# westlake-repl/Adapter4Rec

Hardware: NVIDIA B200
Metric: train user-sequences/s (SASRec + BERT-base LoRA r=8 adapter-tuning step: fwd+bwd+allreduce+Adam) (higher is better)
Workload: dtype bf16

## Files before the change

adapter4rec_b200/csrc/attention_small.cu:

```cuda
#include "a4r_common.cuh"
#include "mma_sync.cuh"

namespace {

constexpr int LP = 32;
constexpr int WARPS_PER_CTA = 4;

struct AttnParams {
  const __nv_bfloat16* qkv;
  __nv_bfloat16* out;
  const __nv_bfloat16* dout;
  const void* mask;
  int64_t ld_qkv, ld_out, mask_ld;
  int N, L, heads;
  int mask_dtype;
  const int32_t* cu_seqlens;
  int causal;
  float scale, mask_neg;
  uint32_t drop_thr16;
  float drop_scale;
  uint64_t drop_seed, drop_offset;
};

A4R_DEVICE void prob_dropout(float (&s)[2][4][4], const AttnParams& p, int n, int h, int lane) {
  const int g = lane >> 2, t = lane & 3;
  const uint64_t base = p.drop_offset + (static_cast<uint64_t>(n) * p.heads + h) * (32 * 8);
  const uint64_t seed = rng_seed(p.drop_seed);
#pragma unroll
  for (int mt = 0; mt < 2; ++mt)
#pragma unroll
    for (int hh = 0; hh < 2; ++hh) {
      const int i = mt * 16 + hh * 8 + g;
#pragma unroll
      for (int np = 0; np < 2; ++np) {
        const uint64_t r = rng64(seed, base + static_cast<uint64_t>(i) * 8 + np * 4 + t);
#pragma unroll
        for (int q = 0; q < 2; ++q)
#pragma unroll
          for (int e = 0; e < 2; ++e) {
            float& x = s[mt][np * 2 + q][hh * 2 + e];
            x = rng_keep(r, q * 2 + e, p.drop_thr16) ? x * p.drop_scale : 0.0f;
          }
      }
    }
}

template <int COLS>
struct Tile {
  static constexpr int kChunks = COLS / 8;
  static constexpr int kBytes = LP * COLS * 2;
  A4R_DEVICE static uint32_t off(int row, int chunk) {
    const int x = COLS == 64 ? row : (row >> 1);
    return static_cast<uint32_t>(row * COLS * 2 + (((chunk ^ x) & (kChunks - 1)) << 4));
  }
};

template <int COLS>
A4R_DEVICE void load_a(uint32_t (&a)[4], uint32_t base, int m0, int k0, int lane) {
  const int mi = lane >> 3, r = lane & 7;
  const int row = m0 + r + ((mi & 1) << 3);
  const int chunk = (k0 >> 3) + (mi >> 1);
  ldsm_x4(a, base + Tile<COLS>::off(row, chunk));
}
template <int COLS>
A4R_DEVICE void load_a_t(uint32_t (&a)[4], uint32_t base, int m0, int k0, int lane) {
  const int mi = lane >> 3, r = lane & 7;
  const int row = k0 + r + ((mi >> 1) << 3);
  const int chunk = (m0 >> 3) + (mi & 1);
  ldsm_x4_t(a, base + Tile<COLS>::off(row, chunk));
}
template <int COLS>
A4R_DEVICE void load_b_nk(uint32_t (&b)[4], uint32_t base, int n0, int k0, int lane) {
  const int mi = lane >> 3, r = lane & 7;
  const int row = n0 + r + ((mi >> 1) << 3);
  const int chunk = (k0 >> 3) + (mi & 1);
  ldsm_x4(b, base + Tile<COLS>::off(row, chunk));
}
template <int COLS>
A4R_DEVICE void load_b_kn(uint32_t (&b)[4], uint32_t base, int n0, int k0, int lane) {
  const int mi = lane >> 3, r = lane & 7;
  const int row = k0 + r + ((mi & 1) << 3);
  const int chunk = (n0 >> 3) + (mi >> 1);
  ldsm_x4_t(b, base + Tile<COLS>::off(row, chunk));
}

template <int DH>
A4R_DEVICE void load_tile(uint8_t* tile, const __nv_bfloat16* g, int64_t ld, int L, int lane) {
  constexpr int CH = DH / 8;
  const uint32_t base = smem_u32(tile);
#pragma unroll
  for (int i = lane; i < LP * CH; i += 32) {
    const int row = i / CH, ch = i % CH;
    const bool ok = row < L;
    const __nv_bfloat16* src = g + (ok ? static_cast<int64_t>(row) * ld + ch * 8 : 0);
    const int sz = ok ? 16 : 0;
    asm volatile("cp.async.cg.shared.global [%0], [%1], 16, %2;" ::"r"(base + Tile<DH>::off(row, ch)), "l"(src), "r"(sz)
                 : "memory");
  }
}
A4R_DEVICE void cp_async_wait_all() { asm volatile("cp.async.wait_all;" ::: "memory"); }
template <int DH>
A4R_DEVICE void store_tile(const uint8_t* tile, __nv_bfloat16* g, int64_t ld, int L, int lane) {
  constexpr int CH = DH / 8;
#pragma unroll
  for (int i = lane; i < LP * CH; i += 32) {
    const int row = i / CH, ch = i % CH;
    if (row < L) st_na_v4(g + static_cast<int64_t>(row) * ld + ch * 8, *reinterpret_cast<const uint4*>(tile + Tile<DH>::off(row, ch)));
  }
}
template <int COLS, int NT>
A4R_DEVICE void acc_to_tile(uint8_t* tile, const float (&acc)[2][NT][4], float s0a, float s0b, float s1a, float s1b, int lane) {
  const int g = lane >> 2, t = lane & 3;
#pragma unroll
  for (int mt = 0; mt < 2; ++mt) {
    const float sa = mt == 0 ? s0a : s1a, sb = mt == 0 ? s0b : s1b;
#pragma unroll
    for (int nt = 0; nt < NT; ++nt) {
      const int r0 = mt * 16 + g, col = nt * 8 + 2 * t;
      *reinterpret_cast<uint32_t*>(tile + Tile<COLS>::off(r0, col >> 3) + (col & 7) * 2) =
          pack_bf16x2(acc[mt][nt][0] * sa, acc[mt][nt][1] * sa);
      *reinterpret_cast<uint32_t*>(tile + Tile<COLS>::off(r0 + 8, col >> 3) + (col & 7) * 2) =
          pack_bf16x2(acc[mt][nt][2] * sb, acc[mt][nt][3] * sb);
    }
  }
}

struct SeqSpan {
  int64_t row0, mask0;
  int L;
};
A4R_DEVICE SeqSpan seq_span(const AttnParams& p, int n) {
  SeqSpan s;
  if (p.cu_seqlens != nullptr) {
    const int a = __ldg(p.cu_seqlens + n), b = __ldg(p.cu_seqlens + n + 1);
    s.row0 = a, s.mask0 = a, s.L = b - a;
  } else {
    s.row0 = static_cast<int64_t>(n) * p.L, s.mask0 = static_cast<int64_t>(n) * p.mask_ld, s.L = p.L;
  }
  return s;
}
A4R_DEVICE bool key_valid(const AttnParams& p, const SeqSpan& sq, int j) {
  if (p.mask_dtype == 1) return reinterpret_cast<const int64_t*>(p.mask)[sq.mask0 + j] != 0;
  if (p.mask_dtype == 2) return reinterpret_cast<const float*>(p.mask)[sq.mask0 + j] != 0.0f;
  return true;
}

template <int DH>
A4R_DEVICE void scores_softmax(float (&s)[2][4][4], uint32_t sQ, uint32_t sK, const AttnParams& p, int L, int lane,
                               uint32_t keymask_bits) {
#pragma unroll
  for (int mt = 0; mt < 2; ++mt)
#pragma unroll
    for (int nt = 0; nt < 4; ++nt)
#pragma unroll
      for (int e = 0; e < 4; ++e) s[mt][nt][e] = 0.0f;
#pragma unroll
  for (int k0 = 0; k0 < DH; k0 += 16) {
    uint32_t a0[4], a1[4];
    load_a<DH>(a0, sQ, 0, k0, lane);
    load_a<DH>(a1, sQ, 16, k0, lane);
#pragma unroll
    for (int np = 0; np < 2; ++np) {
      uint32_t b[4];
      load_b_nk<DH>(b, sK, np * 16, k0, lane);
      const uint32_t b0[2] = {b[0], b[1]}, b1[2] = {b[2], b[3]};
      mma_bf16_16816(s[0][np * 2], a0, b0);
      mma_bf16_16816(s[0][np * 2 + 1], a0, b1);
      mma_bf16_16816(s[1][np * 2], a1, b0);
      mma_bf16_16816(s[1][np * 2 + 1], a1, b1);
    }
  }
  const int g = lane >> 2, t = lane & 3;
  float colneg[4][2];
#pragma unroll
  for (int nt = 0; nt < 4; ++nt)
#pragma unroll
    for (int e = 0; e < 2; ++e) {
      const int j = nt * 8 + 2 * t + e;
      colneg[nt][e] = j >= L ? -INFINITY : (((keymask_bits >> j) & 1u) ? 0.0f : p.mask_neg);
    }
#pragma unroll
  for (int mt = 0; mt < 2; ++mt) {
#pragma unroll
    for (int h = 0; h < 2; ++h) {
      const int i = mt * 16 + h * 8 + g;
      float mx = -INFINITY;
#pragma unroll
      for (int nt = 0; nt < 4; ++nt)
#pragma unroll
        for (int e = 0; e < 2; ++e) {
          float v = fmaf(s[mt][nt][h * 2 + e], p.scale, colneg[nt][e]);
          if (p.causal && nt * 8 + 2 * t + e > i && colneg[nt][e] == 0.0f) v += p.mask_neg;
          s[mt][nt][h * 2 + e] = v;
          mx = fmaxf(mx, v);
        }
      mx = fmaxf(mx, __shfl_xor_sync(0xffffffffu, mx, 1));
      mx = fmaxf(mx, __shfl_xor_sync(0xffffffffu, mx, 2));
      float sum = 0.0f;
#pragma unroll
      for (int nt = 0; nt < 4; ++nt)
#pragma unroll
        for (int e = 0; e < 2; ++e) {
          const float ex = __expf(s[mt][nt][h * 2 + e] - mx);
          s[mt][nt][h * 2 + e] = ex;
          sum += ex;
        }
      sum += __shfl_xor_sync(0xffffffffu, sum, 1);
      sum += __shfl_xor_sync(0xffffffffu, sum, 2);
      const float inv = 1.0f / sum;
#pragma unroll
      for (int nt = 0; nt < 4; ++nt)
#pragma unroll
        for (int e = 0; e < 2; ++e) s[mt][nt][h * 2 + e] *= inv;
    }
  }
}

A4R_DEVICE uint32_t build_keymask(const AttnParams& p, const SeqSpan& sq, int lane) {
  const bool ok = lane < sq.L ? key_valid(p, sq, lane) : false;
  return __ballot_sync(0xffffffffu, ok);
}

A4R_DEVICE void acc_to_a(uint32_t (&a)[4], const float (&c0)[4], const float (&c1)[4]) {
  a[0] = pack_bf16x2(c0[0], c0[1]);
  a[1] = pack_bf16x2(c0[2], c0[3]);
  a[2] = pack_bf16x2(c1[0], c1[1]);
  a[3] = pack_bf16x2(c1[2], c1[3]);
}

template <int DH>
__global__ void __launch_bounds__(WARPS_PER_CTA * 32, 3) attn_fwd_kernel(const AttnParams p) {
  extern __shared__ __align__(128) uint8_t smem_attn[];
  constexpr int TB = Tile<DH>::kBytes;
  const int warp = threadIdx.x >> 5, lane = threadIdx.x & 31;
  uint8_t* my = smem_attn + warp * 3 * TB;
  const int64_t total = static_cast<int64_t>(p.N) * p.heads;
  for (int64_t w = static_cast<int64_t>(blockIdx.x) * WARPS_PER_CTA + warp; w < total;
       w += static_cast<int64_t>(gridDim.x) * WARPS_PER_CTA) {
    const int n = static_cast<int>(w / p.heads), h = static_cast<int>(w % p.heads);
    const int64_t Hd = static_cast<int64_t>(p.heads) * DH;
    const SeqSpan sq = seq_span(p, n);
    const __nv_bfloat16* q = p.qkv + sq.row0 * p.ld_qkv + h * DH;
    load_tile<DH>(my, q, p.ld_qkv, sq.L, lane);
    load_tile<DH>(my + TB, q + Hd, p.ld_qkv, sq.L, lane);
    load_tile<DH>(my + 2 * TB, q + 2 * Hd, p.ld_qkv, sq.L, lane);
    const uint32_t km = build_keymask(p, sq, lane);
    cp_async_wait_all();
    __syncwarp();
    const uint32_t sQ = smem_u32(my), sK = sQ + TB, sV = sK + TB;
    float s[2][4][4];
    scores_softmax<DH>(s, sQ, sK, p, sq.L, lane, km);
    if (p.drop_thr16 != 0) prob_dropout(s, p, n, h, lane);
    float o[2][DH / 8][4];
#pragma unroll
    for (int mt = 0; mt < 2; ++mt)
#pragma unroll
      for (int nt = 0; nt < DH / 8; ++nt)
#pragma unroll
        for (int e = 0; e < 4; ++e) o[mt][nt][e] = 0.0f;
#pragma unroll
    for (int ks = 0; ks < 2; ++ks) {
      uint32_t a0[4], a1[4];
      acc_to_a(a0, s[0][2 * ks], s[0][2 * ks + 1]);
      acc_to_a(a1, s[1][2 * ks], s[1][2 * ks + 1]);
#pragma unroll
      for (int np = 0; np < DH / 16; ++np) {
        uint32_t b[4];
        load_b_kn<DH>(b, sV, np * 16, ks * 16, lane);
        const uint32_t b0[2] = {b[0], b[1]}, b1[2] = {b[2], b[3]};
        mma_bf16_16816(o[0][np * 2], a0, b0);
        mma_bf16_16816(o[0][np * 2 + 1], a0, b1);
        mma_bf16_16816(o[1][np * 2], a1, b0);
        mma_bf16_16816(o[1][np * 2 + 1], a1, b1);
      }
    }
    __syncwarp();
    acc_to_tile<DH, DH / 8>(my, o, 1.f, 1.f, 1.f, 1.f, lane);
    __syncwarp();
    store_tile<DH>(my, p.out + sq.row0 * p.ld_out + h * DH, p.ld_out, sq.L, lane);
    __syncwarp();
  }
}

template <int DH>
__global__ void __launch_bounds__(WARPS_PER_CTA * 32) attn_bwd_kernel(const AttnParams p) {
  extern __shared__ __align__(128) uint8_t smem_attn[];
  constexpr int TB = Tile<DH>::kBytes;
  constexpr int PB = Tile<32>::kBytes;
  const int warp = threadIdx.x >> 5, lane = threadIdx.x & 31;
  uint8_t* my = smem_attn + warp * (4 * TB + 2 * PB);
  const int64_t total = static_cast<int64_t>(p.N) * p.heads;
  for (int64_t w = static_cast<int64_t>(blockIdx.x) * WARPS_PER_CTA + warp; w < total;
       w += static_cast<int64_t>(gridDim.x) * WARPS_PER_CTA) {
    const int n = static_cast<int>(w / p.heads), h = static_cast<int>(w % p.heads);
    const int64_t Hd = static_cast<int64_t>(p.heads) * DH;
    const SeqSpan sq = seq_span(p, n);
    const __nv_bfloat16* q = p.qkv + sq.row0 * p.ld_qkv + h * DH;
    uint8_t *tQ = my, *tK = my + TB, *tV = my + 2 * TB, *tdO = my + 3 * TB, *tP = my + 4 * TB, *tdS = tP + PB;
    load_tile<DH>(tQ, q, p.ld_qkv, sq.L, lane);
    load_tile<DH>(tK, q + Hd, p.ld_qkv, sq.L, lane);
    load_tile<DH>(tV, q + 2 * Hd, p.ld_qkv, sq.L, lane);
    load_tile<DH>(tdO, p.dout + sq.row0 * p.ld_out + h * DH, p.ld_out, sq.L, lane);
    const uint32_t km = build_keymask(p, sq, lane);
    cp_async_wait_all();
    __syncwarp();
    const uint32_t sQ = smem_u32(tQ), sK = smem_u32(tK), sV = smem_u32(tV), sdO = smem_u32(tdO), sP = smem_u32(tP),
                   sdS = smem_u32(tdS);
    float s[2][4][4];
    scores_softmax<DH>(s, sQ, sK, p, sq.L, lane, km);
    float dp[2][4][4];
#pragma unroll
    for (int mt = 0; mt < 2; ++mt)
#pragma unroll
      for (int nt = 0; nt < 4; ++nt)
#pragma unroll
        for (int e = 0; e < 4; ++e) dp[mt][nt][e] = 0.0f;
#pragma unroll
    for (int k0 = 0; k0 < DH; k0 += 16) {
      uint32_t a0[4], a1[4];
      load_a<DH>(a0, sdO, 0, k0, lane);
      load_a<DH>(a1, sdO, 16, k0, lane);
#pragma unroll
      for (int np = 0; np < 2; ++np) {
        uint32_t b[4];
        load_b_nk<DH>(b, sV, np * 16, k0, lane);
        const uint32_t b0[2] = {b[0], b[1]}, b1[2] = {b[2], b[3]};
        mma_bf16_16816(dp[0][np * 2], a0, b0);
        mma_bf16_16816(dp[0][np * 2 + 1], a0, b1);
        mma_bf16_16816(dp[1][np * 2], a1, b0);
        mma_bf16_16816(dp[1][np * 2 + 1], a1, b1);
      }
    }
    float sd[2][4][4];
#pragma unroll
    for (int mt = 0; mt < 2; ++mt)
#pragma unroll
      for (int nt = 0; nt < 4; ++nt)
#pragma unroll
        for (int e = 0; e < 4; ++e) sd[mt][nt][e] = s[mt][nt][e];
    if (p.drop_thr16 != 0) {
      prob_dropout(sd, p, n, h, lane);
#pragma unroll
      for (int mt = 0; mt < 2; ++mt)
#pragma unroll
        for (int nt = 0; nt < 4; ++nt)
#pragma unroll
          for (int e = 0; e < 4; ++e) dp[mt][nt][e] = (sd[mt][nt][e] != 0.0f) ? dp[mt][nt][e] * p.drop_scale : 0.0f;
    }
#pragma unroll
    for (int mt = 0; mt < 2; ++mt)
#pragma unroll
      for (int hh = 0; hh < 2; ++hh) {
        float d = 0.0f;
#pragma unroll
        for (int nt = 0; nt < 4; ++nt)
#pragma unroll
          for (int e = 0; e < 2; ++e) d += s[mt][nt][hh * 2 + e] * dp[mt][nt][hh * 2 + e];
        d += __shfl_xor_sync(0xffffffffu, d, 1);
        d += __shfl_xor_sync(0xffffffffu, d, 2);
#pragma unroll
        for (int nt = 0; nt < 4; ++nt)
#pragma unroll
          for (int e = 0; e < 2; ++e)
            dp[mt][nt][hh * 2 + e] = s[mt][nt][hh * 2 + e] * (dp[mt][nt][hh * 2 + e] - d) * p.scale;
      }
    acc_to_tile<32, 4>(tP, sd, 1.f, 1.f, 1.f, 1.f, lane);
    acc_to_tile<32, 4>(tdS, dp, 1.f, 1.f, 1.f, 1.f, lane);
    __syncwarp();
    float acc[2][DH / 8][4];
#pragma unroll
    for (int mt = 0; mt < 2; ++mt)
#pragma unroll
      for (int nt = 0; nt < DH / 8; ++nt)
#pragma unroll
        for (int e = 0; e < 4; ++e) acc[mt][nt][e] = 0.0f;
#pragma unroll
    for (int ks = 0; ks < 2; ++ks) {
      uint32_t a0[4], a1[4];
      acc_to_a(a0, dp[0][2 * ks], dp[0][2 * ks + 1]);
      acc_to_a(a1, dp[1][2 * ks], dp[1][2 * ks + 1]);
#pragma unroll
      for (int np = 0; np < DH / 16; ++np) {
        uint32_t b[4];
        load_b_kn<DH>(b, sK, np * 16, ks * 16, lane);
        const uint32_t b0[2] = {b[0], b[1]}, b1[2] = {b[2], b[3]};
        mma_bf16_16816(acc[0][np * 2], a0, b0);
        mma_bf16_16816(acc[0][np * 2 + 1], a0, b1);
        mma_bf16_16816(acc[1][np * 2], a1, b0);
        mma_bf16_16816(acc[1][np * 2 + 1], a1, b1);
      }
    }
    float dk[2][DH / 8][4], dv[2][DH / 8][4];
#pragma unroll
    for (int mt = 0; mt < 2; ++mt)
#pragma unroll
      for (int nt = 0; nt < DH / 8; ++nt)
#pragma unroll
        for (int e = 0; e < 4; ++e) dk[mt][nt][e] = dv[mt][nt][e] = 0.0f;
#pragma unroll
    for (int ks = 0; ks < 2; ++ks) {
      uint32_t a0[4], a1[4], p0[4], p1[4];
      load_a_t<32>(a0, sdS, 0, ks * 16, lane);
      load_a_t<32>(a1, sdS, 16, ks * 16, lane);
      load_a_t<32>(p0, sP, 0, ks * 16, lane);
      load_a_t<32>(p1, sP, 16, ks * 16, lane);
#pragma unroll
      for (int np = 0; np < DH / 16; ++np) {
        uint32_t b[4];
        load_b_kn<DH>(b, sQ, np * 16, ks * 16, lane);
        const uint32_t b0[2] = {b[0], b[1]}, b1[2] = {b[2], b[3]};
        mma_bf16_16816(dk[0][np * 2], a0, b0);
        mma_bf16_16816(dk[0][np * 2 + 1], a0, b1);
        mma_bf16_16816(dk[1][np * 2], a1, b0);
        mma_bf16_16816(dk[1][np * 2 + 1], a1, b1);
        uint32_t c[4];
        load_b_kn<DH>(c, sdO, np * 16, ks * 16, lane);
        const uint32_t c0[2] = {c[0], c[1]}, c1[2] = {c[2], c[3]};
        mma_bf16_16816(dv[0][np * 2], p0, c0);
        mma_bf16_16816(dv[0][np * 2 + 1], p0, c1);
        mma_bf16_16816(dv[1][np * 2], p1, c0);
        mma_bf16_16816(dv[1][np * 2 + 1], p1, c1);
      }
    }
    __syncwarp();
    acc_to_tile<DH, DH / 8>(tQ, acc, 1.f, 1.f, 1.f, 1.f, lane);
    acc_to_tile<DH, DH / 8>(tK, dk, 1.f, 1.f, 1.f, 1.f, lane);
    acc_to_tile<DH, DH / 8>(tV, dv, 1.f, 1.f, 1.f, 1.f, lane);
    __syncwarp();
    __nv_bfloat16* dq = p.out + sq.row0 * p.ld_qkv + h * DH;
    store_tile<DH>(tQ, dq, p.ld_qkv, sq.L, lane);
    store_tile<DH>(tK, dq + Hd, p.ld_qkv, sq.L, lane);
    store_tile<DH>(tV, dq + 2 * Hd, p.ld_qkv, sq.L, lane);
    __syncwarp();
  }
}

int check_common(const a4r_attn_args* a) {
  A4R_CHECK_ARG(a != nullptr, "attention: args is NULL");
  A4R_CHECK_ARG(a->qkv && a->out, "attention: qkv/out must be non-NULL");
  A4R_CHECK_ARG(a->L >= 1 && a->L <= LP, "attention_small: L must be in [1,32] (got %lld)", (long long)a->L);
  A4R_CHECK_ARG(a->head_dim == 32 || a->head_dim == 64, "attention_small: head_dim must be 32 or 64");
  A4R_CHECK_ARG(a->heads >= 1 && a->N >= 0, "attention: bad heads/N");
  A4R_CHECK_ARG(a->ld_qkv >= 3 * a->heads * a->head_dim && a->ld_qkv % 8 == 0, "attention: bad ld_qkv");
  A4R_CHECK_ARG(a->ld_out >= a->heads * a->head_dim && a->ld_out % 8 == 0, "attention: bad ld_out");
  A4R_CHECK_ARG(a4r_aligned16(a->qkv) && a4r_aligned16(a->out), "attention: pointers must be 16B aligned");
  A4R_CHECK_ARG(a->mask_dtype >= 0 && a->mask_dtype <= 2, "attention: mask_dtype must be 0,1,2");
  if (a->mask_dtype != 0)
    A4R_CHECK_ARG(a->mask != nullptr && (a->cu_seqlens != nullptr || a->mask_ld >= a->L), "attention: bad mask/mask_ld");
  A4R_CHECK_ARG(a->dropout_p >= 0.0f && a->dropout_p < 1.0f, "attention: dropout_p must be in [0,1)");
  return a4r_device_check();
}

AttnParams to_params(const a4r_attn_args* a) {
  AttnParams p;
  p.qkv = static_cast<const __nv_bfloat16*>(a->qkv);
  p.out = static_cast<__nv_bfloat16*>(a->out);
  p.dout = static_cast<const __nv_bfloat16*>(a->dout);
  p.mask = a->mask;
  p.ld_qkv = a->ld_qkv;
  p.ld_out = a->ld_out;
  p.mask_ld = a->mask_ld;
  p.N = static_cast<int>(a->N);
  p.L = static_cast<int>(a->L);
  p.cu_seqlens = a->cu_seqlens;
  p.heads = static_cast<int>(a->heads);
  p.mask_dtype = a->mask_dtype;
  p.causal = a->causal;
  p.scale = a->scale;
  p.mask_neg = a->mask_neg;
  p.drop_thr16 = static_cast<uint32_t>(a->dropout_p * 65536.0f + 0.5f);
  p.drop_scale = 65536.0f / static_cast<float>(65536u - p.drop_thr16);
  p.drop_seed = a->dropout_seed;
  p.drop_offset = a->dropout_offset;
  return p;
}

template <typename K>
int launch(K kernel, int smem, const AttnParams& p, cudaStream_t stream, bool* attr_done) {
  if (!*attr_done) {
    A4R_CUDA_OK(cudaFuncSetAttribute(kernel, cudaFuncAttributeMaxDynamicSharedMemorySize, smem));
    *attr_done = true;
  }
  const int64_t total = static_cast<int64_t>(p.N) * p.heads;
  int64_t blocks = (total + WARPS_PER_CTA - 1) / WARPS_PER_CTA;
  const int64_t cap = static_cast<int64_t>(a4r_num_sms()) * 8;
  if (blocks > cap) blocks = cap;
  kernel<<<static_cast<int>(blocks), WARPS_PER_CTA * 32, smem, stream>>>(p);
  A4R_LAUNCH_OK();
  a4r_count_launch(1);
  return A4R_OK;
}

}

extern "C" int a4r_attn_small_fwd(const a4r_attn_args* a, a4r_stream_t stream) {
  int rc = check_common(a);
  if (rc != A4R_OK) return rc;
  if (a->N == 0) return A4R_OK;
  const AttnParams p = to_params(a);
  static bool done64 = false, done32 = false;
  if (a->head_dim == 64)
    return launch(attn_fwd_kernel<64>, WARPS_PER_CTA * 3 * Tile<64>::kBytes, p, static_cast<cudaStream_t>(stream), &done64);
  return launch(attn_fwd_kernel<32>, WARPS_PER_CTA * 3 * Tile<32>::kBytes, p, static_cast<cudaStream_t>(stream), &done32);
}

extern "C" int a4r_attn_small_bwd(const a4r_attn_args* a, a4r_stream_t stream) {
  int rc = check_common(a);
  if (rc != A4R_OK) return rc;
  A4R_CHECK_ARG(a->dout != nullptr && a4r_aligned16(a->dout), "attention bwd: dout missing or unaligned");
  if (a->N == 0) return A4R_OK;
  const AttnParams p = to_params(a);
  static bool done64 = false, done32 = false;
  if (a->head_dim == 64)
    return launch(attn_bwd_kernel<64>, WARPS_PER_CTA * (4 * Tile<64>::kBytes + 2 * Tile<32>::kBytes), p,
                  static_cast<cudaStream_t>(stream), &done64);
  return launch(attn_bwd_kernel<32>, WARPS_PER_CTA * (4 * Tile<32>::kBytes + 2 * Tile<32>::kBytes), p,
                static_cast<cudaStream_t>(stream), &done32);
}
```

Baseline: 2003.

## Cut attention backward register and smem pressure, size grids by measured occupancy

The backward kernel now computes dQ, dK and dV one after another with a single reused accumulator, storing each through the K tile. This replaces three live accumulators and lowers register pressure. For head_dim 64 the P/dS tiles alias the V tile, which shrinks per-warp shared memory. Warps per CTA and min-CTA launch bounds change separately for forward (2, 8) and backward (7, 2), and the grid cap now comes from cudaOccupancyMaxActiveBlocksPerMultiprocessor instead of a fixed 8 per SM. The trade is serialized stores and extra warp syncs in backward, and possible register spills under the tighter forward bound.

```diff
diff --git a/adapter4rec_b200/csrc/attention_small.cu b/adapter4rec_b200/csrc/attention_small.cu
--- a/adapter4rec_b200/csrc/attention_small.cu
+++ b/adapter4rec_b200/csrc/attention_small.cu
@@ -4,7 +4,8 @@
 namespace {
 
 constexpr int LP = 32;
-constexpr int WARPS_PER_CTA = 4;
+constexpr int FWD_WARPS = 2, FWD_MIN_CTAS = 8;
+constexpr int BWD_WARPS = 7, BWD_MIN_CTAS = 2;
 
 struct AttnParams {
   const __nv_bfloat16* qkv;
@@ -229,14 +230,14 @@
 }
 
 template <int DH>
-__global__ void __launch_bounds__(WARPS_PER_CTA * 32, 3) attn_fwd_kernel(const AttnParams p) {
+__global__ void __launch_bounds__(FWD_WARPS * 32, FWD_MIN_CTAS) attn_fwd_kernel(const AttnParams p) {
   extern __shared__ __align__(128) uint8_t smem_attn[];
   constexpr int TB = Tile<DH>::kBytes;
   const int warp = threadIdx.x >> 5, lane = threadIdx.x & 31;
   uint8_t* my = smem_attn + warp * 3 * TB;
   const int64_t total = static_cast<int64_t>(p.N) * p.heads;
-  for (int64_t w = static_cast<int64_t>(blockIdx.x) * WARPS_PER_CTA + warp; w < total;
-       w += static_cast<int64_t>(gridDim.x) * WARPS_PER_CTA) {
+  for (int64_t w = static_cast<int64_t>(blockIdx.x) * FWD_WARPS + warp; w < total;
+       w += static_cast<int64_t>(gridDim.x) * FWD_WARPS) {
     const int n = static_cast<int>(w / p.heads), h = static_cast<int>(w % p.heads);
     const int64_t Hd = static_cast<int64_t>(p.heads) * DH;
     const SeqSpan sq = seq_span(p, n);
@@ -283,20 +284,26 @@
 }
 
 template <int DH>
-__global__ void __launch_bounds__(WARPS_PER_CTA * 32) attn_bwd_kernel(const AttnParams p) {
+__host__ __device__ constexpr int bwd_warp_bytes() {
+  return 4 * Tile<DH>::kBytes + (2 * Tile<32>::kBytes <= Tile<DH>::kBytes ? 0 : 2 * Tile<32>::kBytes);
+}
+template <int DH>
+__global__ void __launch_bounds__(BWD_WARPS * 32, BWD_MIN_CTAS) attn_bwd_kernel(const AttnParams p) {
   extern __shared__ __align__(128) uint8_t smem_attn[];
   constexpr int TB = Tile<DH>::kBytes;
   constexpr int PB = Tile<32>::kBytes;
   const int warp = threadIdx.x >> 5, lane = threadIdx.x & 31;
-  uint8_t* my = smem_attn + warp * (4 * TB + 2 * PB);
+  uint8_t* my = smem_attn + warp * bwd_warp_bytes<DH>();
   const int64_t total = static_cast<int64_t>(p.N) * p.heads;
-  for (int64_t w = static_cast<int64_t>(blockIdx.x) * WARPS_PER_CTA + warp; w < total;
-       w += static_cast<int64_t>(gridDim.x) * WARPS_PER_CTA) {
+  for (int64_t w = static_cast<int64_t>(blockIdx.x) * BWD_WARPS + warp; w < total;
+       w += static_cast<int64_t>(gridDim.x) * BWD_WARPS) {
     const int n = static_cast<int>(w / p.heads), h = static_cast<int>(w % p.heads);
     const int64_t Hd = static_cast<int64_t>(p.heads) * DH;
     const SeqSpan sq = seq_span(p, n);
     const __nv_bfloat16* q = p.qkv + sq.row0 * p.ld_qkv + h * DH;
-    uint8_t *tQ = my, *tK = my + TB, *tV = my + 2 * TB, *tdO = my + 3 * TB, *tP = my + 4 * TB, *tdS = tP + PB;
+    uint8_t *tQ = my, *tK = my + TB, *tV = my + 2 * TB, *tdO = my + 3 * TB;
+    uint8_t* tP = 2 * PB <= TB ? tV : my + 4 * TB;
+    uint8_t* tdS = tP + PB;
     load_tile<DH>(tQ, q, p.ld_qkv, sq.L, lane);
     load_tile<DH>(tK, q + Hd, p.ld_qkv, sq.L, lane);
     load_tile<DH>(tV, q + 2 * Hd, p.ld_qkv, sq.L, lane);
@@ -364,6 +371,7 @@
           for (int e = 0; e < 2; ++e)
             dp[mt][nt][hh * 2 + e] = s[mt][nt][hh * 2 + e] * (dp[mt][nt][hh * 2 + e] - d) * p.scale;
       }
+    __syncwarp();
     acc_to_tile<32, 4>(tP, sd, 1.f, 1.f, 1.f, 1.f, lane);
     acc_to_tile<32, 4>(tdS, dp, 1.f, 1.f, 1.f, 1.f, lane);
     __syncwarp();
@@ -390,47 +398,63 @@
         mma_bf16_16816(acc[1][np * 2 + 1], a1, b1);
       }
     }
-    float dk[2][DH / 8][4], dv[2][DH / 8][4];
+    __nv_bfloat16* dq = p.out + sq.row0 * p.ld_qkv + h * DH;
+    __syncwarp();
+    acc_to_tile<DH, DH / 8>(tK, acc, 1.f, 1.f, 1.f, 1.f, lane);
+    __syncwarp();
+    store_tile<DH>(tK, dq, p.ld_qkv, sq.L, lane);
 #pragma unroll
     for (int mt = 0; mt < 2; ++mt)
 #pragma unroll
       for (int nt = 0; nt < DH / 8; ++nt)
 #pragma unroll
-        for (int e = 0; e < 4; ++e) dk[mt][nt][e] = dv[mt][nt][e] = 0.0f;
+        for (int e = 0; e < 4; ++e) acc[mt][nt][e] = 0.0f;
 #pragma unroll
     for (int ks = 0; ks < 2; ++ks) {
-      uint32_t a0[4], a1[4], p0[4], p1[4];
+      uint32_t a0[4], a1[4];
       load_a_t<32>(a0, sdS, 0, ks * 16, lane);
       load_a_t<32>(a1, sdS, 16, ks * 16, lane);
-      load_a_t<32>(p0, sP, 0, ks * 16, lane);
-      load_a_t<32>(p1, sP, 16, ks * 16, lane);
 #pragma unroll
       for (int np = 0; np < DH / 16; ++np) {
         uint32_t b[4];
         load_b_kn<DH>(b, sQ, np * 16, ks * 16, lane);
         const uint32_t b0[2] = {b[0], b[1]}, b1[2] = {b[2], b[3]};
-        mma_bf16_16816(dk[0][np * 2], a0, b0);
-        mma_bf16_16816(dk[0][np * 2 + 1], a0, b1);
-        mma_bf16_16816(dk[1][np * 2], a1, b0);
-        mma_bf16_16816(dk[1][np * 2 + 1], a1, b1);
+        mma_bf16_16816(acc[0][np * 2], a0, b0);
+        mma_bf16_16816(acc[0][np * 2 + 1], a0, b1);
+        mma_bf16_16816(acc[1][np * 2], a1, b0);
+        mma_bf16_16816(acc[1][np * 2 + 1], a1, b1);
+      }
+    }
+    __syncwarp();
+    acc_to_tile<DH, DH / 8>(tK, acc, 1.f, 1.f, 1.f, 1.f, lane);
+    __syncwarp();
+    store_tile<DH>(tK, dq + Hd, p.ld_qkv, sq.L, lane);
+#pragma unroll
+    for (int mt = 0; mt < 2; ++mt)
+#pragma unroll
+      for (int nt = 0; nt < DH / 8; ++nt)
+#pragma unroll
+        for (int e = 0; e < 4; ++e) acc[mt][nt][e] = 0.0f;
+#pragma unroll
+    for (int ks = 0; ks < 2; ++ks) {
+      uint32_t p0[4], p1[4];
+      load_a_t<32>(p0, sP, 0, ks * 16, lane);
+      load_a_t<32>(p1, sP, 16, ks * 16, lane);
+#pragma unroll
+      for (int np = 0; np < DH / 16; ++np) {
         uint32_t c[4];
         load_b_kn<DH>(c, sdO, np * 16, ks * 16, lane);
         const uint32_t c0[2] = {c[0], c[1]}, c1[2] = {c[2], c[3]};
-        mma_bf16_16816(dv[0][np * 2], p0, c0);
-        mma_bf16_16816(dv[0][np * 2 + 1], p0, c1);
-        mma_bf16_16816(dv[1][np * 2], p1, c0);
-        mma_bf16_16816(dv[1][np * 2 + 1], p1, c1);
-      }
-    }
-    __syncwarp();
-    acc_to_tile<DH, DH / 8>(tQ, acc, 1.f, 1.f, 1.f, 1.f, lane);
-    acc_to_tile<DH, DH / 8>(tK, dk, 1.f, 1.f, 1.f, 1.f, lane);
-    acc_to_tile<DH, DH / 8>(tV, dv, 1.f, 1.f, 1.f, 1.f, lane);
-    __syncwarp();
-    __nv_bfloat16* dq = p.out + sq.row0 * p.ld_qkv + h * DH;
-    store_tile<DH>(tQ, dq, p.ld_qkv, sq.L, lane);
-    store_tile<DH>(tK, dq + Hd, p.ld_qkv, sq.L, lane);
-    store_tile<DH>(tV, dq + 2 * Hd, p.ld_qkv, sq.L, lane);
+        mma_bf16_16816(acc[0][np * 2], p0, c0);
+        mma_bf16_16816(acc[0][np * 2 + 1], p0, c1);
+        mma_bf16_16816(acc[1][np * 2], p1, c0);
+        mma_bf16_16816(acc[1][np * 2 + 1], p1, c1);
+      }
+    }
+    __syncwarp();
+    acc_to_tile<DH, DH / 8>(tK, acc, 1.f, 1.f, 1.f, 1.f, lane);
+    __syncwarp();
+    store_tile<DH>(tK, dq + 2 * Hd, p.ld_qkv, sq.L, lane);
     __syncwarp();
   }
 }
@@ -476,16 +500,19 @@
 }
 
 template <typename K>
-int launch(K kernel, int smem, const AttnParams& p, cudaStream_t stream, bool* attr_done) {
-  if (!*attr_done) {
+int launch(K kernel, int warps, int smem, const AttnParams& p, cudaStream_t stream, int* ctas_per_sm) {
+  if (*ctas_per_sm == 0) {
     A4R_CUDA_OK(cudaFuncSetAttribute(kernel, cudaFuncAttributeMaxDynamicSharedMemorySize, smem));
-    *attr_done = true;
+    int nb = 0;
+    A4R_CUDA_OK(cudaOccupancyMaxActiveBlocksPerMultiprocessor(&nb, kernel, warps * 32, smem));
+    A4R_CHECK_ARG(nb >= 1, "attention_small: a CTA does not fit on an SM");
+    *ctas_per_sm = nb;
   }
   const int64_t total = static_cast<int64_t>(p.N) * p.heads;
-  int64_t blocks = (total + WARPS_PER_CTA - 1) / WARPS_PER_CTA;
-  const int64_t cap = static_cast<int64_t>(a4r_num_sms()) * 8;
+  int64_t blocks = (total + warps - 1) / warps;
+  const int64_t cap = static_cast<int64_t>(a4r_num_sms()) * *ctas_per_sm;
   if (blocks > cap) blocks = cap;
-  kernel<<<static_cast<int>(blocks), WARPS_PER_CTA * 32, smem, stream>>>(p);
+  kernel<<<static_cast<int>(blocks), warps * 32, smem, stream>>>(p);
   A4R_LAUNCH_OK();
   a4r_count_launch(1);
   return A4R_OK;
@@ -498,10 +525,10 @@
   if (rc != A4R_OK) return rc;
   if (a->N == 0) return A4R_OK;
   const AttnParams p = to_params(a);
-  static bool done64 = false, done32 = false;
-  if (a->head_dim == 64)
-    return launch(attn_fwd_kernel<64>, WARPS_PER_CTA * 3 * Tile<64>::kBytes, p, static_cast<cudaStream_t>(stream), &done64);
-  return launch(attn_fwd_kernel<32>, WARPS_PER_CTA * 3 * Tile<32>::kBytes, p, static_cast<cudaStream_t>(stream), &done32);
+  static int occ64 = 0, occ32 = 0;
+  const cudaStream_t s = static_cast<cudaStream_t>(stream);
+  if (a->head_dim == 64) return launch(attn_fwd_kernel<64>, FWD_WARPS, FWD_WARPS * 3 * Tile<64>::kBytes, p, s, &occ64);
+  return launch(attn_fwd_kernel<32>, FWD_WARPS, FWD_WARPS * 3 * Tile<32>::kBytes, p, s, &occ32);
 }
 
 extern "C" int a4r_attn_small_bwd(const a4r_attn_args* a, a4r_stream_t stream) {
@@ -510,10 +537,8 @@
   A4R_CHECK_ARG(a->dout != nullptr && a4r_aligned16(a->dout), "attention bwd: dout missing or unaligned");
   if (a->N == 0) return A4R_OK;
   const AttnParams p = to_params(a);
-  static bool done64 = false, done32 = false;
-  if (a->head_dim == 64)
-    return launch(attn_bwd_kernel<64>, WARPS_PER_CTA * (4 * Tile<64>::kBytes + 2 * Tile<32>::kBytes), p,
-                  static_cast<cudaStream_t>(stream), &done64);
-  return launch(attn_bwd_kernel<32>, WARPS_PER_CTA * (4 * Tile<32>::kBytes + 2 * Tile<32>::kBytes), p,
-                static_cast<cudaStream_t>(stream), &done32);
-}
+  static int occ64 = 0, occ32 = 0;
+  const cudaStream_t s = static_cast<cudaStream_t>(stream);
+  if (a->head_dim == 64) return launch(attn_bwd_kernel<64>, BWD_WARPS, BWD_WARPS * bwd_warp_bytes<64>(), p, s, &occ64);
+  return launch(attn_bwd_kernel<32>, BWD_WARPS, BWD_WARPS * bwd_warp_bytes<32>(), p, s, &occ32);
+}
```

New measurement: 2012 (median of 6 runs). Within noise of the previous version (+0.4%).
